# go-distributed/gossip_simulator

Measured on AMD Instinct MI355X. Metric: gossip messages delivered/sec (node) at N=1e9; rounds-to-coverage parity, higher is better.
Workload: dtype u32; 1 GPU; C5-reference-model: single push-flood broadcast per GPU; n=1000000000, fanout=5, fanin=6, delaylow=10, delayhigh=20, ticks=290, status=quiescent, parallelism=trials1

## Files before the change

gossip_simulator_amd/csrc/gs_ctx.cpp:

```cpp
#include "gs_ctx.h"

namespace gs {

namespace {

uint32_t ring_slots(const gs_params& p) { return p.delay_high > 2 ? (uint32_t)p.delay_high : 2u; }

uint32_t ceil_log2(uint64_t x) {
  uint32_t b = 0;
  while ((1ull << b) < x) ++b;
  return b;
}

int check_params(const gs_params* p, bool rumor_trials, std::string& why) {
  if (!p) { why = "params is NULL"; return GS_EINVAL; }
  if (p->n == 0) { why = "n must be >= 1 (simulator.go:240 panics on rand.Intn(0))"; return GS_EINVAL; }
  if (p->n > 0x7FFFFFFFull) { why = "n must be < 2^31"; return GS_EINVAL; }
  if (p->delay_high <= p->delay_low) {
    why = "delayhigh must exceed delaylow (simulator.go:167 panics on rand.Intn(<=0))";
    return GS_EINVAL;
  }
  if (p->fanout < 0 || p->fanin < 0 || p->fanout > 255 || p->fanin > 255) {
    why = "fanout/fanin must be in [0, 255]";
    return GS_EINVAL;
  }
  if (ring_slots(*p) > 4096) { why = "delayhigh must be <= 4096"; return GS_EINVAL; }
  if (p->model > GS_MODEL_RUMOR) {
    why = "model must be GS_MODEL_FLOOD, GS_MODEL_PUSHPULL or GS_MODEL_RUMOR";
    return GS_EINVAL;
  }
  if (p->model == GS_MODEL_RUMOR && (p->rumor_k < 1 || p->rumor_k > 255)) {
    why = "GS_MODEL_RUMOR needs 1 <= rumor_k <= 255, not " + std::to_string(p->rumor_k);
    return GS_EINVAL;
  }
  if (p->model == GS_MODEL_RUMOR && (p->rumor_mode & ~(GS_RUMOR_BLIND | GS_RUMOR_COIN | GS_RUMOR_PULL))) {
    why = "GS_MODEL_RUMOR: rumor_mode " + std::to_string(p->rumor_mode) +
          " has a bit that is none of GS_RUMOR_BLIND, GS_RUMOR_COIN, GS_RUMOR_PULL";
    return GS_EINVAL;
  }
  if (p->model == GS_MODEL_RUMOR && p->trials > 1 && !rumor_trials) {
    why = "GS_MODEL_RUMOR with trials > 1: the rumor model runs one trial per context (gs_create_trials makes a batch)";
    return GS_EINVAL;
  }
  if (p->trials > 1 && ((uint64_t)p->trials << std::max<uint32_t>(kFineLog, ceil_log2(p->n))) > 0x7FFFFFFFull) {
    why = "trials x 2^ceil(log2 n) must be < 2^31 (batch fewer trials per context)";
    return GS_EINVAL;
  }
  return GS_OK;
}

bool alloc_trial_rows(gs_ctx* c, size_t tb, size_t cb) {
  return dev_malloc((void**)&c->bt.d_tstat, tb) == hipSuccess &&
         hipHostMalloc((void**)&c->bt.h_tstat, tb) == hipSuccess && grow(c->bt.chk, cb);
}

void release_trials(gs_ctx* c) {
  if (c->bt.d_tstat) (void)dev_free(c->bt.d_tstat);
  if (c->bt.h_tstat) (void)hipHostFree(c->bt.h_tstat);
  release(c->bt.chk);
}

int alloc_window(gs_ctx* c) {
  const DevState& s = c->st;
  WinState& w = c->ws;
  w.n = s.n;
  w.W = s.W;
  w.nfine = (uint32_t)((s.n + kFineNodes - 1) >> kFineLog);
  w.ncoarse = (w.nfine + 255) / 256;
  w.R = s.R;
  w.delay_low = s.delay_low;
  w.delay_span = s.delay_span;
  w.kd = s.kd;
  w.kc = s.kc;
  w.key = s.key;
  w.base = (uint32_t)c->lo;
  w.tlog = c->tlog;
  w.tmask = c->tlog >= 32 ? ~0u : (1u << c->tlog) - 1;
  w.tnodes = c->trials > 1 && c->tlog <= kCoarseShift && !c->shard ? (uint32_t)c->p.n : 0u;
  w.G = c->G;
  w.rank = c->rank;
  w.seg_per = (uint32_t)c->seg_per;
  w.csub = kCoarseSub;
  w.noxcd = getenv("GS_PART2_NOXCD") ? 1u : 0u;
  {
    const char* xp = getenv("GS_XPAIR");
    w.nopair = xp && atoi(xp) == 0 ? 1u : 0u;
  }
  w.ccap_end = nullptr;
  w.csrc = nullptr;
  if (c->shard) {
    w.owner = 1;
    w.obins = 256 / c->G;
    w.oseg_q = (uint32_t)(c->seg_per >> kFineLog);
    w.oseg_magic = 0xFFFFFFFFu / w.oseg_q;
    if (dev_malloc(&c->wn.d_rtab, kRtabWords * 8) != hipSuccess ||
        hipHostMalloc((void**)&c->wn.h_rtab, kRtabWords * 8) != hipSuccess)
      return fail(c, GS_ENOMEM, "cannot allocate the shard's receive layout");
  }
  auto al = [](size_t b) { return (b + 255) & ~(size_t)255; };
  const size_t units = (size_t)kMaxWindow * w.nfine + 1;
  const size_t b_fc = al((size_t)w.R * w.nfine * 4), b_units = al(units * 8),
               b_small = al(kRegions * 8) * 2 + al((kRegions + 1) * 8) + al((kRegions + 1) * 4) + al(kMaxWindow * 8),
               b_fhist = al(((size_t)w.ncoarse * 256 + 1) * 8), b_fbase = al(((size_t)w.nfine + 1) * 8),
               b_ffill = al((size_t)w.nfine * 8),
               b_sst = al((size_t)kStatShards * kMaxWindow * kStatFields * 8),
               b_rlcnt = al((size_t)w.nfine * 4),
               b_tsum = al((size_t)w.ncoarse * kMaxWindow * 8) + al(((size_t)w.ncoarse + 1) * 8);
  const size_t total = b_fc + 2 * b_units + b_small + b_fhist + b_fbase + b_ffill + b_sst + b_rlcnt + b_tsum;
  if (dev_malloc(&c->wn.d_win, total) != hipSuccess)
    return fail(c, GS_ENOMEM, "cannot allocate window-engine buffers");
  const size_t flist = (size_t)w.R * w.nfine * kFineNodes * 2;
  if (dev_malloc(&c->wn.d_flist, flist) != hipSuccess)
    return fail(c, GS_ENOMEM, "cannot allocate " + std::to_string(flist >> 20) + " MiB of fire lists");
  char* q = (char*)c->wn.d_win;
  w.fcount = (uint32_t*)q; q += b_fc;
  w.usize = (unsigned long long*)q; q += b_units;
  w.unit_off = (unsigned long long*)q; q += b_units;
  w.chist = (unsigned long long*)q; q += al(kRegions * 8);
  w.cfill = (unsigned long long*)q; q += al(kRegions * 8);
  w.ccap = (unsigned long long*)q; q += al((kRegions + 1) * 8);
  w.tprefix = (uint32_t*)q; q += al((kRegions + 1) * 4);
  w.tfires = (unsigned long long*)q;
  q = (char*)c->wn.d_win + b_fc + 2 * b_units + b_small;
  w.fhist = (unsigned long long*)q; q += b_fhist;
  w.fstart = (unsigned long long*)q; q += b_fbase;
  w.ffill = (unsigned long long*)q; q += b_ffill;
  w.sstats = (unsigned long long*)q; q += b_sst;
  w.rlcnt = (uint32_t*)q; q += b_rlcnt;
  w.tsum = (unsigned long long*)q; q += al((size_t)w.ncoarse * kMaxWindow * 8);
  w.toff = (unsigned long long*)q; q += al(((size_t)w.ncoarse + 1) * 8);
  if (dev_malloc(&c->wn.d_rlmsg, (size_t)w.nfine * kRolledCap * 4) != hipSuccess)
    return fail(c, GS_ENOMEM, "cannot allocate the rolled-receipt lists");
  w.rlmsg = (uint32_t*)c->wn.d_rlmsg;
  w.dbg = nullptr;
  if (getenv("GS_STAMPS") && dev_malloc(&w.dbg, kDbgWords * 8) == hipSuccess)
    (void)hipMemset(w.dbg, 0, kDbgWords * 8);
  w.flist = (uint16_t*)c->wn.d_flist;
  c->wn.fcount_bytes = (size_t)w.R * w.nfine * 4;
  if (hipMemsetAsync(c->wn.d_win, 0, total, c->stream) != hipSuccess)
    return fail(c, GS_EDEVICE, "memset of window buffers failed");
  c->wn.misc_words = std::max<size_t>(4096, (size_t)c->G * kMaxWindow + 64);
  if (hipHostMalloc((void**)&c->wn.h_cap, (kRegions + 1) * 8) != hipSuccess ||
      hipHostMalloc((void**)&c->wn.h_misc, c->wn.misc_words * 8) != hipSuccess ||
      hipHostMalloc((void**)&c->wn.h_err, 64) != hipSuccess)
    return fail(c, GS_ENOMEM, "cannot allocate pinned window buffers");
  if (c->trials > 1) {
    if (!alloc_trial_rows(c, (size_t)c->trials * kMaxWindow * kTStatFields * 4, 0))
      return fail(c, GS_ENOMEM, "cannot allocate per-trial counters");
    w.tstat = c->bt.d_tstat;
  }
  return GS_OK;
}

void release_window(gs_ctx* c) {
  WinEngine& e = c->wn;
  for (void* p : {e.d_win, e.d_flist, e.d_rlmsg, (void*)e.d_rtab, (void*)c->ws.dbg})
    if (p) (void)dev_free(p);
  for (Buf* b : {&e.gmap, &e.cmsg, &e.fmsg, &e.tmp}) release(*b);
  for (void* p : {(void*)e.h_cap, (void*)e.h_misc, (void*)e.h_err, (void*)e.h_rtab})
    if (p) (void)hipHostFree(p);
}

int ctx_setup(gs_ctx* c, const gs_params* params, int device, bool shard, uint32_t G, uint32_t rank,
              std::string& why) {
  c->p = *params;
  c->p.device = device;
  c->dev = device;
  int ndev = 0;
  if (hipGetDeviceCount(&ndev) != hipSuccess || ndev <= 0) {
    why = "no HIP device visible (libgossip_hip needs an MI355X)";
    return GS_EDEVICE;
  }
  if (c->dev < 0 || c->dev >= ndev) {
    why = "device " + std::to_string(c->dev) + " out of range (" + std::to_string(ndev) + " visible)";
    return GS_EDEVICE;
  }
  hipDeviceProp_t prop;
  if (hipSetDevice(c->dev) != hipSuccess || hipGetDeviceProperties(&prop, c->dev) != hipSuccess ||
      strncmp(prop.gcnArchName, "gfx950", 6) != 0) {
    why = "device " + std::to_string(c->dev) + " is not gfx950";
    return GS_EDEVICE;
  }
  if (hipStreamCreateWithFlags(&c->own, hipStreamNonBlocking) != hipSuccess) {
    why = "cannot create a stream";
    return GS_EDEVICE;
  }
  c->stream = c->own;
  DevState& s = c->st;
  const uint32_t stride0 = (uint32_t)std::max(c->p.fanout, c->p.fanin);
  c->pp = c->p.model == GS_MODEL_PUSHPULL;
  c->rumor = c->p.model == GS_MODEL_RUMOR;
  c->pp_l2_only = (c->p.flags & GS_FLAG_PP_L2_ONLY) != 0;
  c->trials = std::max<uint32_t>(1, c->p.trials);
  c->ntot = c->p.n;
  if (c->trials > 1) {
    c->tlog = std::max<uint32_t>(kFineLog, ceil_log2(c->p.n));
    c->ntot = (uint64_t)c->trials << c->tlog;
  }
  c->shard = shard;
  c->G = G;
  c->rank = rank;
  if (shard && c->rumor) {
    why = "GS_MODEL_RUMOR runs on one device: no node-range shards";
    return GS_EINVAL;
  }
  if (shard) {
    if (c->pp && !pp_rslot_packed(stride0)) {
      why = "push-pull node-range shards need rows of at most 16 slots (bottom-up rounds)";
      return GS_EINVAL;
    }
    c->seg_per = (((c->p.n + G - 1) / G) + kFineNodes - 1) & ~(uint64_t)(kFineNodes - 1);
// ... 486 lines not shown
```

gossip_simulator_amd/csrc/gs_internal.h:

```cpp
#pragma once
#include <stdint.h>
#include <hip/hip_runtime.h>

#include <algorithm>
#include <vector>

#include "gs_devmem.h"
#include "gs_rng.h"

namespace gs {

inline uint32_t grid_for(uint64_t items, uint32_t per_block, uint32_t cap) {
  return (uint32_t)std::min<uint64_t>((items + per_block - 1) / per_block, cap);
}

constexpr uint32_t kWave = 64;
constexpr uint32_t kChunkNodesLog = 12;
constexpr uint32_t kChunkWords = 64;
constexpr uint32_t kShards = 32;
constexpr uint32_t kCounterStride = 16;
constexpr uint32_t kStatFields = 8;
constexpr uint32_t kStatSlots = 4096;
constexpr uint32_t kListCap = 1024;
constexpr uint32_t kTickBlock = 256;
constexpr uint32_t kTickGridMax = 2048;

enum Stat : uint32_t {
  ST_FIRED = 0, ST_SENT = 1, ST_MSGS = 2, ST_RECV = 3, ST_CRASH = 4, ST_SCHED = 5,
  ST_ERR = 6, ST_RSVD = 7
};

enum Mode : int {
  MODE_FLOOD = 0,
  MODE_COUNT = 1,
  MODE_RESOLVE = 2
};

struct DevState {
  const uint8_t* deg;
  const uint32_t* ids;
  unsigned long long* recv;
  unsigned long long* crash;
  uint32_t* rollw;
  uint32_t* cnt;
  unsigned long long* ring;
  uint32_t* cflag;
  uint32_t* clist;
  uint32_t* ccount;
  unsigned long long* stats;
  uint32_t* err;
  unsigned long long* grecv;
  unsigned long long* gcrash;
  uint64_t gbase;
  uint64_t n, W;
  uint32_t C, CS, R, stride;
  uint32_t stride_magic;
  int32_t delay_low;
  uint32_t delay_span;
  int32_t kd, kc;
  int32_t check_crashed;
  int32_t sharded;
  uint32_t lo, hi;
  uint32_t chunk_lo, chunk_hi;
  Key key;
};

constexpr uint32_t kFineLog = 14;
constexpr uint32_t kFineNodes = 1u << kFineLog;
constexpr uint32_t kCoarseShift = kFineLog + 8;
constexpr uint32_t kMaxWindow = 16;
constexpr uint32_t kCoarseSub = 8;
constexpr uint32_t kRegions = 256 * kCoarseSub;
constexpr uint32_t kWinMaxRing = 256;
constexpr uint32_t kWinMaxStride = 32;
constexpr uint32_t kEmptyMsg = 0xFFFFFFFFu;
constexpr uint32_t kSrcShift = 56;
constexpr unsigned long long kSrcMask = (1ull << kSrcShift) - 1;
#ifndef GS_PART_TILE
#define GS_PART_TILE 16384
#endif
constexpr uint32_t kPartTile = GS_PART_TILE;
constexpr uint32_t kRolledCap = 1024;
constexpr uint32_t kBitTicks = 10;
constexpr uint32_t kXRoundNodes = 2048;
constexpr uint32_t kWinSlotsPerBucket = 1u << 16;

struct WinCtl {
  uint32_t t, L, tnext, tend;
  uint32_t poll, pbase, stop, lmax;
  unsigned long long Tn, T;
  unsigned long long recv, crashed, pending, cover, max_ticks;
  unsigned long long cmsg_cap, fmsg_cap;
  unsigned long long xs_cap, xr_cap;
};
constexpr uint32_t kStageWords = 8 + 16 * 8;

struct WinState {
  const uint8_t* deg;
  const uint32_t* ids;
  unsigned long long* recv;
  unsigned long long* crash;
  uint32_t* rollw;
  uint32_t* rlmsg;
  uint32_t* rlcnt;
  unsigned long long* stats;
  uint32_t* err;
  uint32_t* fcount;
  uint16_t* flist;
  unsigned long long* usize;
  unsigned long long* unit_off;
  unsigned long long* tfires;
  uint32_t* gmap;
  const uint32_t* pk;
  uint32_t noxcd;
  uint32_t nopair;
  uint32_t* cmsg;
  uint32_t* fmsg;
  unsigned long long* chist;
  unsigned long long* ccap;
  const unsigned long long* ccap_end;
  unsigned long long* cfill;
  uint32_t* tprefix;
  unsigned long long* fhist;
  unsigned long long* fstart;
  unsigned long long* ffill;
  unsigned long long* tsum;
  unsigned long long* toff;
  unsigned long long* sstats;
  unsigned long long* dbg;
  uint32_t* tstat;
  uint32_t tofs;
  WinCtl* ctl;
  unsigned long long* stage;
  uint32_t lstride;
  uint32_t slots;
  uint32_t csub;
  const uint32_t* const* csrc;
  uint32_t owner;
  uint32_t obins;
  uint32_t oseg_q, oseg_magic;
  uint32_t abort_on_err;
  uint32_t G, rank;
  uint32_t seg_per;
  uint32_t dd;
  uint32_t guard;
  uint32_t solo;
  unsigned long long* gcnt;
  unsigned long long* glay;
  unsigned long long* wstat;
  uint64_t nglob;
  uint64_t n, W;
  uint32_t nfine, ncoarse, R, stride, stride_magic;
  int32_t delay_low;
  uint32_t delay_span;
  int32_t kd, kc;
  uint32_t base;
  uint32_t tlog, tmask;
  uint32_t tnodes;
  Key key;
};
constexpr uint32_t kStatShards = 32;
constexpr uint32_t kStampPhases = 10;
constexpr uint32_t kXStamp0 = 2 * kStampPhases;
constexpr uint32_t kDbgWords = kXStamp0 + 8;
enum TStat : uint32_t { TS_FIRED = 0, TS_SENT = 1, TS_DEAD = 2, TS_RECV = 3, TS_CRASH = 4, TS_HOT = 5 };
constexpr uint32_t kTStatFields = 8;

__host__ __device__ __forceinline__ void node_key(uint32_t tlog, uint32_t tmask, const Key& key,
                                                  uint64_t g, uint32_t kind, uint32_t& node,
                                                  uint32_t& c3) {
  node = (uint32_t)(g & tmask);
  c3 = ctr3(kind, key.trial + (uint32_t)(g >> tlog));
}

constexpr uint32_t kErrArrivals = 4;
constexpr uint32_t kErrCoarse = 8;
constexpr uint32_t kErrFine = 16;
constexpr uint32_t kErrAbort = 32;
constexpr uint32_t kErrNoMem = 64;
constexpr uint32_t kDDRow = kRegions + 4;
constexpr uint32_t kDDWStat = kMaxWindow * kStatFields + 8;
constexpr size_t kRtabWords = 4 * (kRegions + 1) + 260;
constexpr size_t kRtabTotal = kRtabWords - 1;

hipError_t win_units(const WinState& w, uint32_t t0, uint32_t L, hipStream_t s);
hipError_t win_cut(const WinState& w, unsigned long long budget, hipStream_t s);
hipError_t win_unitscan(const WinState& w, hipStream_t s);
// ... 230 lines not shown
```

gossip_simulator_amd/csrc/gs_win_resolve.hip:

```cpp
#include <algorithm>

#include "gs_win_dev.h"

namespace gs {
namespace {

constexpr uint32_t kResolveMaxBuckets = 256;
constexpr uint32_t kSmallMax = 256;
#ifndef GS_SMALL_BLOCK
#define GS_SMALL_BLOCK 512
#endif
constexpr uint32_t kSmallBlock = GS_SMALL_BLOCK;
#ifndef GS_ROLLED_BLOCK
#define GS_ROLLED_BLOCK 256
#endif
constexpr uint32_t kRolledBlock = GS_ROLLED_BLOCK;

constexpr uint32_t kBitWords = kFineNodes / 32;
struct ResolveLds {
  union {
    struct {
      uint32_t b1[kBitTicks][kBitWords];
      uint2 cr0[kBitWords];
    };
    struct {
      uint32_t cnt[kFineNodes];
      uint32_t recv[kBitWords];
      uint32_t crash[kBitWords];
      uint32_t nrecv[kBitWords];
      uint32_t ncrash[kBitWords];
    };
  };
  uint32_t fc[kWinMaxRing];
  uint32_t st[kMaxWindow][4];
  uint32_t dead[kMaxWindow];
  uint32_t blist[kResolveMaxBuckets];
  unsigned long long bstart[kResolveMaxBuckets];
  uint32_t bcnt[kResolveMaxBuckets];
  uint32_t ndup;
  uint32_t ninf;
  uint32_t err;
  uint32_t nb;
  uint32_t cls;
  unsigned long long stamp[2][kStampPhases];
  unsigned long long tlast;
};
static_assert(kBitTicks <= kMaxWindow, "window ticks fit the message format");
static_assert(sizeof(uint32_t) * kFineNodes <= sizeof(((ResolveLds*)0)->cnt), "the infection list fits");

__device__ __forceinline__ void stamp(const WinState& w, ResolveLds& sm, uint32_t i) {
  if (w.dbg && threadIdx.x == 0) {
    const unsigned long long t = __builtin_amdgcn_s_memtime();
    if (i) sm.stamp[sm.cls][i] += t - sm.tlast;
    sm.tlast = t;
  }
}

#if defined(GS_RESOLVE_PROBE) && GS_RESOLVE_PROBE == 1
#define GS_RESOLVE_CR0(loc) make_uint2(0u, 0u)
#else
#define GS_RESOLVE_CR0(loc) sm.cr0[(loc) >> 5]
#endif


__device__ __forceinline__ void resolve_node(const WinState& w, ResolveLds& sm, uint32_t f,
                                             uint32_t loc, uint32_t kk, uint32_t ones, uint32_t t,
                                             uint32_t& cm, uint32_t& cr, uint32_t& cc, uint32_t& cs) {
  const uint32_t bit = 1u << (loc & 31), wi = loc >> 5;
  if (sm.crash[wi] & bit) return;
  const uint64_t g = (uint64_t)w.base + (f << kFineLog) + loc;
  uint32_t u, c3order;
  node_key(w.tlog, w.tmask, w.key, g, K_ORDER, u, c3order);
  const uint32_t pos = ones ? first_crash(u, t, kk, ones, c3order, w.key.k0, w.key.k1) : kk + 1;
  cm += pos <= kk ? pos : kk;
  if (pos > 1 && !(sm.recv[wi] & bit)) {
    atomicOr(&sm.recv[wi], bit);
    ++cr;
    uint32_t c3delay;
    node_key(w.tlog, w.tmask, w.key, g, K_DELAY, u, c3delay);
    const uint32_t off = fire_offset(w.delay_low, w.delay_span,
                                     philox(u, t, 0, c3delay, w.key.k0, w.key.k1).x);
    const uint32_t s = (t + off) % w.R;
    const uint32_t at = atomicAdd(&sm.fc[s], 1u);
    w.flist[((size_t)s * w.nfine + f) * kFineNodes + at] = (uint16_t)loc;
    ++cs;
  }
  if (pos <= kk) {
    atomicOr(&sm.crash[wi], bit);
    ++cc;
  }
}

template <class Src>
__device__ __forceinline__ void resolve_tick(const WinState& w, ResolveLds& sm, uint32_t f,
                                             const Src& src, uint32_t lo, uint32_t hi, uint32_t k,
                                             uint32_t t) {
  const uint32_t tid = threadIdx.x;
  for (uint32_t p = lo + tid; p < hi; p += kResolveBlock) {
    const uint32_t m = src[p];
    if (msg_tick(m) != k) continue;
    const uint32_t old = atomicAdd(&sm.cnt[msg_loc(m)], 1u + (((m >> kRoll0Fine) & 1u) << 16));
    if ((old & 0xFFFFu) == 0xFFFFu) sm.err = 1;
  }
  __syncthreads();
  uint32_t arr = 0, cm = 0, cr = 0, cc = 0, cs = 0;
  for (uint32_t p = lo + tid; p < hi; p += kResolveBlock) {
    const uint32_t m = src[p];
    if (msg_tick(m) != k) continue;
    const uint32_t loc = msg_loc(m);
    const uint32_t kk = atomicExch(&sm.cnt[loc], 0u);
    arr += kk & 0xFFFFu;
    if (kk) resolve_node(w, sm, f, loc, kk & 0xFFFFu, kk >> 16, t, cm, cr, cc, cs);
  }
  if (arr != cm) atomicAdd(&sm.st[k][0], arr - cm);
  if (cr) atomicAdd(&sm.st[k][1], cr);
  if (cc) atomicAdd(&sm.st[k][2], cc);
  (void)cs;
  __syncthreads();
}

__device__ __forceinline__ void flush_counts(const WinState& w, ResolveLds& sm, uint32_t (&acc_ni)[kBitTicks / 2],
                                             uint32_t L, uint32_t trial) {
#pragma unroll
  for (uint32_t k = 0; k < kBitTicks; ++k) {
    if (k >= L) continue;
    const uint32_t sr = wave_sum((acc_ni[k / 2] >> (16 * (k & 1))) & 0xFFFFu);
    if (lane_id() == 0 && sr) atomicAdd(&sm.st[k][1], sr);
  }
#pragma unroll
  for (uint32_t k = 0; k < kBitTicks / 2; ++k) acc_ni[k] = 0;
  __syncthreads();
  const uint32_t tid = threadIdx.x;
  if (tid < L * 3) {
    const uint32_t k = tid / 3, fld = tid - k * 3;
    const uint32_t v = sm.st[k][fld];
    unsigned long long* row = shard_row(w, k);
    if (v && fld == 0) atomicAdd(&row[ST_MSGS], 0ull - (unsigned long long)v);
    if (v && fld == 1) {
      atomicAdd(&row[ST_RECV], (unsigned long long)v);
      atomicAdd(&row[ST_SCHED], (unsigned long long)v);
    }
    if (v && fld == 2) atomicAdd(&row[ST_CRASH], (unsigned long long)v);
    if (v && trial != ~0u) atomicAdd(&w.tstat[((size_t)trial * kMaxWindow + w.tofs + k) * kTStatFields + TS_DEAD + fld], v);
    sm.st[k][fld] = 0;
  }
  __syncthreads();
}

__device__ __forceinline__ void resolve_body(const WinState& w, uint32_t t0, uint32_t L) {
  __shared__ ResolveLds sm;
  const uint32_t tid = threadIdx.x, G = gridDim.x;
  L = win_live(w, t0, L);
  if (!L) return;
  static_assert(kBitWords == kResolveBlock, "one bit word per thread");
  static_assert(kWinMaxRing <= kResolveBlock, "one ring slot per thread");
  if (tid < kMaxWindow * 4) (&sm.st[0][0])[tid] = 0;
  if (tid == 0) { sm.nb = 0; sm.cls = 0; }
  if (tid < 2 * kStampPhases) (&sm.stamp[0][0])[tid] = 0;
  __syncthreads();
  {
    const uint32_t f = blockIdx.x + tid * G;
    const unsigned long long fl = tid < kResolveMaxBuckets && f < w.nfine ? w.ffill[f] : 0ull;
    const bool ne = fl > kSmallMax;
    const uint32_t at = wave_append(&sm.nb, ne);
    if (ne) {
      sm.blist[at] = f;
      sm.bstart[at] = w.fstart[f];
      sm.bcnt[at] = (uint32_t)fl;
    }
  }
  __syncthreads();
  const uint32_t nb = sm.nb;
  stamp(w, sm, 0);
  uint32_t fB = 0, MB = 0;
  unsigned long long mbB = 0;
  auto next_bucket = [&](uint32_t j) { fB = sm.blist[j]; mbB = sm.bstart[j]; MB = sm.bcnt[j]; };
  if (nb > 0) next_bucket(0);
  uint32_t* rwg = (uint32_t*)w.recv;
  uint32_t* cwg = (uint32_t*)w.crash;
  uint32_t acc_ni[kBitTicks / 2];
#pragma unroll
  for (uint32_t k = 0; k < kBitTicks / 2; ++k) acc_ni[k] = 0;
  static_assert(kBitTicks % 2 == 0 && 32 * kResolveMaxBuckets < 65536, "two 16-bit counts per register");
  constexpr uint32_t kU = 8;
  constexpr uint32_t kBatch = kResolveBlock * kU;
  auto ld = [&](const uint32_t* gm, uint32_t M, uint32_t p0, uint32_t (&m)[kU]) {
#pragma unroll
    for (uint32_t u = 0; u < kU; ++u) {
      const uint32_t p = p0 + u * kResolveBlock + tid;
      m[u] = *reinterpret_cast<const uint32_t*>(reinterpret_cast<const char*>(gm) + ((p < M ? p : M - 1) << 2));
    }
  };
  uint32_t pm[kU], p_recv0 = 0, p_crash0 = 0, p_roll0 = 0, p_fcv = 0;
  bool p_in = false;
  auto prefetch = [&](uint32_t f, uint32_t M, unsigned long long mb) {
    const uint64_t wi = ((uint64_t)(f << kFineLog) >> 5) + tid;
    const bool in = wi < w.W * 2;
    const uint64_t wc = in ? wi : w.W * 2 - 1;
    p_in = in;
    p_recv0 = rwg[wc];
    p_crash0 = cwg[wc];
    p_roll0 = w.rollw[wc];
    p_fcv = w.fcount[(size_t)(tid < w.R ? tid : 0u) * w.nfine + f];
    ld(w.fmsg + mb, M, 0, pm);
// ... 94 lines not shown
    if (i + 1 < nb) prefetch(fB, MB, mbB);
    if (tid == 0) w.rlcnt[f] = sm.err == 3 ? 0u : min(sm.ndup, kRolledCap);
    stamp(w, sm, 3);
    uint32_t rw = recv0, cw = crash0;
    if (sm.err != 3) {
      if (tid < L && sm.dead[tid]) atomicAdd(&sm.st[tid][0], sm.dead[tid]);
      uint32_t infk[kBitTicks], ninf = 0;
      const uint32_t plain = ~(crash0 | rollw);
#pragma unroll
      for (uint32_t k = 0; k < kBitTicks; ++k) {
        infk[k] = 0;
        if (k >= L) continue;
        const uint32_t infS = sm.b1[k][tid] & plain & ~rw;
        rw |= infS;
        infk[k] = infS;
      }
      stamp(w, sm, 4);
#pragma unroll
      for (uint32_t k = 0; k < kBitTicks; ++k) {
        const uint32_t ni = __popc(infk[k]);
        acc_ni[k / 2] += ni << (16 * (k & 1));
        ninf += ni;
      }
      stamp(w, sm, 5);
      __syncthreads();
      stamp(w, sm, 6);
      auto bcast = [&](uint32_t x) {
        const uint32_t loc = msg_loc(x), t = t0 + msg_tick(x);
        const uint32_t off = fire_offset(w.delay_low, w.delay_span,
                                         philox(knode0 + loc, t, 0, c3delay, w.key.k0, w.key.k1).x);
        const uint32_t slot = (t + off) % w.R;
        const uint32_t pos = atomicAdd(&sm.fc[slot], 1u);
        w.flist[((size_t)slot * w.nfine + f) * kFineNodes + pos] = (uint16_t)loc;
      };
      uint32_t* inf = &sm.cnt[0];
      {
        uint32_t pre = 0, tot = 0;
#pragma unroll
        for (uint32_t b = 0; b < 9; ++b) {
          const unsigned long long bal = __ballot((ninf >> b) & 1u);
          pre += lanes_below(bal) << b;
          tot += (uint32_t)__popcll(bal) << b;
        }
        uint32_t base = 0;
        if (tot && lane_id() == 0) base = atomicAdd(&sm.ninf, tot);
        uint32_t at = __builtin_amdgcn_readfirstlane(base) + pre;
#pragma unroll
        for (uint32_t k = 0; k < kBitTicks; ++k)
          for (uint32_t x = k < L ? infk[k] : 0u; x; x &= x - 1)
            inf[at++] = (tid * 32 + __builtin_ctz(x)) | (k << kFineLog);
      }
      __syncthreads();
      stamp(w, sm, 7);
      const uint32_t ni_all = sm.ninf;
      for (uint32_t q = tid; q < ni_all; q += kResolveBlock) bcast(inf[q]);
    } else {
      __syncthreads();
      uint4* c4 = reinterpret_cast<uint4*>(sm.cnt);
      for (uint32_t q = tid; q < kFineNodes / 4; q += kResolveBlock) c4[q] = make_uint4(0, 0, 0, 0);
      sm.recv[tid] = recv0;
      sm.crash[tid] = crash0;
      sm.nrecv[tid] = 0;
      sm.ncrash[tid] = 0;
      __syncthreads();
      for (uint32_t k = 0; k < L; ++k) resolve_tick(w, sm, f, gm, 0, M, k, t0 + k);
      rw = sm.recv[tid] | sm.nrecv[tid];
      cw = sm.crash[tid] | sm.ncrash[tid];
      if (tid == 0 && sm.err == 1) atomicOr(w.err, kErrArrivals);
    }
    __syncthreads();
    stamp(w, sm, 8);
    if (in) {
      if (rw != recv0) rwg[wi] = rw;
      if (cw != crash0) cwg[wi] = cw;
    }
    if (tid < w.R) w.fcount[(size_t)tid * w.nfine + f] = sm.fc[tid];
    stamp(w, sm, 9);
    if (w.dbg && tid == 0) sm.stamp[sm.cls][0] += 1;
    if (w.tstat) flush_counts(w, sm, acc_ni, L, (uint32_t)(((uint64_t)w.base + node0) >> w.tlog));
  }
  if (w.dbg && tid < 2 * kStampPhases) atomicAdd(&w.dbg[tid], (&sm.stamp[0][0])[tid]);
  if (!w.tstat) flush_counts(w, sm, acc_ni, L, ~0u);
}
__global__ __launch_bounds__(kResolveBlock, GS_RESOLVE_WAVES) void k_resolve(const WinState w, uint32_t t0, uint32_t L) {
  resolve_body(w, t0, L);
}
__global__ __launch_bounds__(kResolveBlock, GS_RESOLVE_WAVES) void k_resolve_m(const WinState* __restrict__ ws,
                                                                                uint32_t L) {
  resolve_body(ws[blockIdx.y], 0u, L);
}

template <uint32_t E, bool ROLLED>
__device__ __forceinline__ void resolve_small_bucket(const WinState& w, uint32_t t0, uint32_t L, uint32_t f,
                                                     const uint32_t* gm, unsigned long long M,
                                                     uint32_t (*st)[kMaxWindow][4], uint32_t* skw,
                                                     uint32_t* fcw) {
  constexpr uint32_t N = 64 * E;
  const uint32_t lane = threadIdx.x & 63, wv = threadIdx.x >> 6;
  {
    const bool consume = !ROLLED && w.ctl;
    const uint32_t s0 = t0 % w.R;
    for (uint32_t s = lane; s < w.R; s += 64)
      fcw[s] = consume && (s + w.R - s0) % w.R < L ? 0u : w.fcount[(size_t)s * w.nfine + f];
    uint32_t knode0, c3order;
    node_key(w.tlog, w.tmask, w.key, (uint64_t)w.base + (f << kFineLog), K_ORDER, knode0, c3order);
    const uint32_t c3delay = (c3order & 0xFFFFFFu) | (K_DELAY << 24);
    uint32_t key[E];
#pragma unroll
    for (uint32_t r = 0; r < E; ++r) {
      const uint32_t i = lane * E + r;
      key[r] = ~0u;
      if (i < M) {
        const uint32_t m = gm[i];
        key[r] = (msg_loc(m) << 5) | (msg_tick(m) << 1) | ((m >> kRoll0Fine) & 1u);
        if (!ROLLED && ((m >> kRoll0Fine) & 1u)) w.rollw[((f << kFineLog) + msg_loc(m)) >> 5] = 0u;
      }
    }
#pragma unroll
    for (uint32_t k = 2; k <= N; k <<= 1)
#pragma unroll
      for (uint32_t j = k >> 1; j > 0; j >>= 1) {
        if (j >= E) {
#pragma unroll
          for (uint32_t r = 0; r < E; ++r) {
            const uint32_t i = lane * E + r;
            const uint32_t o = __shfl_xor(key[r], j / E, 64);
            const bool keep_min = ((i & j) == 0) == ((i & k) == 0);
            key[r] = keep_min ? min(key[r], o) : max(key[r], o);
          }
        } else {
#pragma unroll
          for (uint32_t r = 0; r < E; ++r) {
            if (r & j) continue;
            const bool up = ((lane * E + r) & k) == 0;
            const uint32_t a = key[r], b = key[r | j];
            key[r] = up ? min(a, b) : max(a, b);
            key[r | j] = up ? max(a, b) : min(a, b);
          }
        }
      }
#pragma unroll
    for (uint32_t r = 0; r < E; ++r) skw[lane * E + r] = key[r];
    wave_lds_sync();
    uint32_t* rwg = (uint32_t*)w.recv;
    uint32_t* cwg = (uint32_t*)w.crash;
    bool any_inf = false;
    uint32_t head = 0;
#pragma unroll
    for (uint32_t r = 0; r < E; ++r) {
      const uint32_t i = lane * E + r;
      if (key[r] != ~0u && !(i > 0 && (skw[i - 1] >> 5) == (key[r] >> 5))) head |= 1u << r;
    }
#pragma unroll 1
    for (uint32_t r = 0; r < E; ++r) {
      if (!((head >> r) & 1u)) continue;
      const uint32_t i = lane * E + r;
      const uint32_t loc = skw[i] >> 5;
      const uint32_t wi = ((f << kFineLog) + loc) >> 5, bit = 1u << (loc & 31), u = knode0 + loc;
      const uint32_t cw = cwg[wi];
      bool rv = (rwg[wi] & bit) != 0, cr = (cw & bit) != 0, inf = false;
      uint32_t tinf = 0;
      for (uint32_t q = i; q < N;) {
        const uint32_t e = skw[q];
        if ((e >> 5) != loc) break;
        const uint32_t k = (e >> 1) & (kMaxWindow - 1), t = t0 + k;
        uint32_t c = 0, ones = 0;
        for (; q < N && (skw[q] >> 1) == (e >> 1); ++q) {
          ++c;
          ones += skw[q] & 1u;
        }
        if (cr) {
          atomicAdd(&st[wv][k][0], c);
// ... 22 lines not shown
        w.flist[((size_t)slot * w.nfine + f) * kFineNodes + pos] = (uint16_t)loc;
      }
    }
    wave_lds_sync();
    if (__ballot(any_inf)) {
      for (uint32_t s = lane; s < w.R; s += 64) w.fcount[(size_t)s * w.nfine + f] = fcw[s];
    } else if (consume && lane < L) {
      w.fcount[(size_t)((t0 + lane) % w.R) * w.nfine + f] = 0;
    }
    if (w.tstat) {
      wave_lds_sync();
      if (lane < L * 3) {
        const uint32_t k = lane / 3, fld = lane - k * 3;
        const uint32_t v = st[wv][k][fld];
        const uint32_t trial = (uint32_t)(((uint64_t)w.base + (f << kFineLog)) >> w.tlog);
        if (v) atomicAdd(&w.tstat[((size_t)trial * kMaxWindow + w.tofs + k) * kTStatFields + TS_DEAD + fld], v);
      }
    }
  }
}

template <bool ROLLED>
__device__ __forceinline__ void resolve_small_body(const WinState& w, uint32_t t0, uint32_t L) {
  constexpr uint32_t kWaves = (ROLLED ? kRolledBlock : kSmallBlock) / 64;
  constexpr uint32_t kEmax = ROLLED ? 16 : 4;
  __shared__ uint32_t st[kWaves][kMaxWindow][4];
  __shared__ uint32_t sk[kWaves][64 * kEmax];
  __shared__ uint32_t fcw[kWaves][kWinMaxRing];
  const uint32_t tid = threadIdx.x, wv = tid >> 6;
  static_assert(kWaves * kMaxWindow * 4 == kWaves * 64, "one counter per thread");
  static_assert(kRolledCap == 64 * 16, "the rolled bodies cover 1..kRolledCap");
  const uint32_t f = __builtin_amdgcn_readfirstlane(blockIdx.x * kWaves + wv);
  unsigned long long M = 0;
  const uint32_t* gm = nullptr;
  if (f < w.nfine) {
    if (ROLLED) {
      M = w.rlcnt[f];
      gm = w.rlmsg + (size_t)f * kRolledCap;
    } else {
      M = w.ffill[f];
      gm = w.fmsg + w.fstart[f];
    }
  }
  L = win_live(w, t0, L);
  if (!L) return;
  (&st[0][0][0])[tid] = 0;
  __syncthreads();
  if (M > 0 && M <= 64) resolve_small_bucket<1, ROLLED>(w, t0, L, f, gm, M, st, sk[wv], fcw[wv]);
  else if (M > 64 && M <= 256) resolve_small_bucket<4, ROLLED>(w, t0, L, f, gm, M, st, sk[wv], fcw[wv]);
  else if (ROLLED && M > 256 && M <= 512)
    resolve_small_bucket<ROLLED ? 8 : 1, ROLLED>(w, t0, L, f, gm, M, st, sk[wv], fcw[wv]);
  else if (ROLLED && M > 512 && M <= kRolledCap)
    resolve_small_bucket<ROLLED ? 16 : 1, ROLLED>(w, t0, L, f, gm, M, st, sk[wv], fcw[wv]);
  if (ROLLED && M && (threadIdx.x & 63) == 0) w.rlcnt[f] = 0;
  if (!ROLLED && w.ctl && !(M > 0 && M <= 256) && f < w.nfine && (threadIdx.x & 63) < L)
    w.fcount[(size_t)((t0 + (threadIdx.x & 63)) % w.R) * w.nfine + f] = 0;
  __syncthreads();
  if (tid < L * 3) {
    const uint32_t k = tid / 3, fld = tid - k * 3;
    uint32_t v = 0;
    for (uint32_t q = 0; q < kWaves; ++q) v += st[q][k][fld];
    unsigned long long* row = shard_row(w, k);
    if (v && fld == 0) atomicAdd(&row[ST_MSGS], 0ull - (unsigned long long)v);
    if (v && fld == 1) {
      atomicAdd(&row[ST_RECV], (unsigned long long)v);
      atomicAdd(&row[ST_SCHED], (unsigned long long)v);
    }
    if (v && fld == 2) atomicAdd(&row[ST_CRASH], (unsigned long long)v);
  }
}
template <bool ROLLED>
__global__ __launch_bounds__(ROLLED ? kRolledBlock : kSmallBlock) void k_resolve_small(const WinState w, uint32_t t0,
                                                                                       uint32_t L) {
  resolve_small_body<ROLLED>(w, t0, L);
}
template <bool ROLLED>
__global__ __launch_bounds__(ROLLED ? kRolledBlock : kSmallBlock) void k_resolve_small_m(
    const WinState* __restrict__ ws, uint32_t L) {
  resolve_small_body<ROLLED>(ws[blockIdx.y], 0u, L);
}

}

hipError_t win_resolve(const WinState& w, uint32_t t0, uint32_t L, hipStream_t s) {
  const uint32_t cus = device_cus();
  static const uint32_t per_cu = [] { const char* e = getenv("GS_RESOLVE_PER_CU"); return e ? (uint32_t)std::max(atoi(e), 1) : 2u; }();
  uint32_t G = std::min<uint32_t>(w.nfine, per_cu * cus);
  G = std::max<uint32_t>(G, (w.nfine + kResolveMaxBuckets - 1) / kResolveMaxBuckets);
  const uint32_t gs = (w.nfine + kSmallBlock / 64 - 1) / (kSmallBlock / 64);
  hipLaunchKernelGGL(k_resolve_small<false>, dim3(gs), dim3(kSmallBlock), 0, s, w, t0, L);
  static_assert(kSmallMax == 64 * 4, "the two bodies cover 1..kSmallMax");
  hipLaunchKernelGGL(k_resolve, dim3(G), dim3(kResolveBlock), 0, s, w, t0, L);
  hipLaunchKernelGGL(k_resolve_small<true>, dim3((w.nfine + kRolledBlock / 64 - 1) / (kRolledBlock / 64)),
                     dim3(kRolledBlock), 0, s, w, t0, L);
  return hipGetLastError();
}

hipError_t win_resolve_g(const WinGroup& g, uint32_t L, hipStream_t s) {
  const uint32_t cus = device_cus();
  uint32_t G = std::min<uint32_t>(g.nfine_max, (2 * cus + g.M - 1) / g.M);
  G = std::max<uint32_t>(G, (g.nfine_max + kResolveMaxBuckets - 1) / kResolveMaxBuckets);
  const uint32_t gs = (g.nfine_max + kSmallBlock / 64 - 1) / (kSmallBlock / 64);
  hipLaunchKernelGGL(k_resolve_small_m<false>, dim3(gs, g.M), dim3(kSmallBlock), 0, s, g.wr, L);
  hipLaunchKernelGGL(k_resolve_m, dim3(G, g.M), dim3(kResolveBlock), 0, s, g.wr, L);
  hipLaunchKernelGGL(k_resolve_small_m<true>, dim3((g.nfine_max + kRolledBlock / 64 - 1) / (kRolledBlock / 64), g.M),
                     dim3(kRolledBlock), 0, s, g.wr, L);
  return hipGetLastError();
}

}
```

Measured before the change: 84.56 billion msgs/s.

## Add slimmer-LDS resolve kernel with overflow fallback to a large-bucket pass

Introduces a new resolve kernel whose shared-memory footprint is trimmed (a smaller infection list unioned with the crash/roll words, dead counts packed into 6-bit fields), so three workgroups fit per CU instead of two. It also prefetches the next bucket's state. Buckets whose duplicate-receipt list overflows are recorded in a new global list and handled by a separate large-bucket kernel running the old per-tick path. This is enabled by default with more blocks per CU. The risks are an extra launch, chunked infection processing when the list exceeds its capacity, and more complex control flow.

```diff
diff --git a/gossip_simulator_amd/csrc/gs_ctx.cpp b/gossip_simulator_amd/csrc/gs_ctx.cpp
--- a/gossip_simulator_amd/csrc/gs_ctx.cpp
+++ b/gossip_simulator_amd/csrc/gs_ctx.cpp
@@ -104,7 +104,7 @@
                b_fhist = al(((size_t)w.ncoarse * 256 + 1) * 8), b_fbase = al(((size_t)w.nfine + 1) * 8),
                b_ffill = al((size_t)w.nfine * 8),
                b_sst = al((size_t)kStatShards * kMaxWindow * kStatFields * 8),
-               b_rlcnt = al((size_t)w.nfine * 4),
+               b_rlcnt = al((size_t)w.nfine * 4) + al(((size_t)w.nfine + 2) * 4),
                b_tsum = al((size_t)w.ncoarse * kMaxWindow * 8) + al(((size_t)w.ncoarse + 1) * 8);
   const size_t total = b_fc + 2 * b_units + b_small + b_fhist + b_fbase + b_ffill + b_sst + b_rlcnt + b_tsum;
   if (dev_malloc(&c->wn.d_win, total) != hipSuccess)
@@ -126,7 +126,8 @@
   w.fstart = (unsigned long long*)q; q += b_fbase;
   w.ffill = (unsigned long long*)q; q += b_ffill;
   w.sstats = (unsigned long long*)q; q += b_sst;
-  w.rlcnt = (uint32_t*)q; q += b_rlcnt;
+  w.rlcnt = (uint32_t*)q; q += al((size_t)w.nfine * 4);
+  w.lgl = (uint32_t*)q; q += al(((size_t)w.nfine + 2) * 4);
   w.tsum = (unsigned long long*)q; q += al((size_t)w.ncoarse * kMaxWindow * 8);
   w.toff = (unsigned long long*)q; q += al(((size_t)w.ncoarse + 1) * 8);
   if (dev_malloc(&c->wn.d_rlmsg, (size_t)w.nfine * kRolledCap * 4) != hipSuccess)
diff --git a/gossip_simulator_amd/csrc/gs_internal.h b/gossip_simulator_amd/csrc/gs_internal.h
--- a/gossip_simulator_amd/csrc/gs_internal.h
+++ b/gossip_simulator_amd/csrc/gs_internal.h
@@ -103,6 +103,7 @@
   uint32_t* rollw;
   uint32_t* rlmsg;
   uint32_t* rlcnt;
+  uint32_t* lgl;
   unsigned long long* stats;
   uint32_t* err;
   uint32_t* fcount;
diff --git a/gossip_simulator_amd/csrc/gs_win_resolve.hip b/gossip_simulator_amd/csrc/gs_win_resolve.hip
--- a/gossip_simulator_amd/csrc/gs_win_resolve.hip
+++ b/gossip_simulator_amd/csrc/gs_win_resolve.hip
@@ -48,7 +48,8 @@
 static_assert(kBitTicks <= kMaxWindow, "window ticks fit the message format");
 static_assert(sizeof(uint32_t) * kFineNodes <= sizeof(((ResolveLds*)0)->cnt), "the infection list fits");
 
-__device__ __forceinline__ void stamp(const WinState& w, ResolveLds& sm, uint32_t i) {
+template <class Lds>
+__device__ __forceinline__ void stamp(const WinState& w, Lds& sm, uint32_t i) {
   if (w.dbg && threadIdx.x == 0) {
     const unsigned long long t = __builtin_amdgcn_s_memtime();
     if (i) sm.stamp[sm.cls][i] += t - sm.tlast;
@@ -119,7 +120,8 @@
   __syncthreads();
 }
 
-__device__ __forceinline__ void flush_counts(const WinState& w, ResolveLds& sm, uint32_t (&acc_ni)[kBitTicks / 2],
+template <class Lds>
+__device__ __forceinline__ void flush_counts(const WinState& w, Lds& sm, uint32_t (&acc_ni)[kBitTicks / 2],
                                              uint32_t L, uint32_t trial) {
 #pragma unroll
   for (uint32_t k = 0; k < kBitTicks; ++k) {
@@ -380,12 +382,299 @@
   if (w.dbg && tid < 2 * kStampPhases) atomicAdd(&w.dbg[tid], (&sm.stamp[0][0])[tid]);
   if (!w.tstat) flush_counts(w, sm, acc_ni, L, ~0u);
 }
-__global__ __launch_bounds__(kResolveBlock, GS_RESOLVE_WAVES) void k_resolve(const WinState w, uint32_t t0, uint32_t L) {
+__global__ __launch_bounds__(kResolveBlock, GS_RESOLVE_WAVES) void k_resolve2(const WinState w, uint32_t t0, uint32_t L) {
   resolve_body(w, t0, L);
 }
-__global__ __launch_bounds__(kResolveBlock, GS_RESOLVE_WAVES) void k_resolve_m(const WinState* __restrict__ ws,
-                                                                                uint32_t L) {
+__global__ __launch_bounds__(kResolveBlock, GS_RESOLVE_WAVES) void k_resolve2_m(const WinState* __restrict__ ws,
+                                                                                 uint32_t L) {
   resolve_body(ws[blockIdx.y], 0u, L);
+}
+
+constexpr uint32_t kInfCap = 6656;
+constexpr uint32_t kResolveWaves3 = 6;
+struct ResolveLds3 {
+  uint32_t b1[kBitTicks][kBitWords];
+  union {
+    uint2 cr0[kBitWords];
+    uint32_t inf[kInfCap];
+  };
+  uint32_t fc[kWinMaxRing];
+  uint32_t st[kMaxWindow][4];
+  uint32_t dead[kMaxWindow];
+  uint32_t blist[kResolveMaxBuckets];
+  unsigned long long bstart[kResolveMaxBuckets];
+  uint32_t bcnt[kResolveMaxBuckets];
+  uint32_t ndup;
+  uint32_t ninf;
+  uint32_t err;
+  uint32_t nb;
+  uint32_t cls;
+  unsigned long long stamp[2][kStampPhases];
+  unsigned long long tlast;
+};
+static_assert(sizeof(ResolveLds3) <= 53 * 1024, "three workgroups per CU");
+static_assert(kBitTicks * 6 <= 64, "6-bit dead counts per tick in one register pair");
+
+__device__ __forceinline__ void resolve3_body(const WinState& w, uint32_t t0, uint32_t L) {
+  __shared__ ResolveLds3 sm;
+  const uint32_t tid = threadIdx.x, G = gridDim.x;
+  L = win_live(w, t0, L);
+  if (!L) return;
+  if (tid < kMaxWindow * 4) (&sm.st[0][0])[tid] = 0;
+  if (tid == 0) { sm.nb = 0; sm.cls = 0; }
+  if (tid < 2 * kStampPhases) (&sm.stamp[0][0])[tid] = 0;
+  __syncthreads();
+  {
+    const uint32_t f = blockIdx.x + tid * G;
+    const unsigned long long fl = tid < kResolveMaxBuckets && f < w.nfine ? w.ffill[f] : 0ull;
+    const bool ne = fl > kSmallMax;
+    const uint32_t at = wave_append(&sm.nb, ne);
+    if (ne) {
+      sm.blist[at] = f;
+      sm.bstart[at] = w.fstart[f];
+      sm.bcnt[at] = (uint32_t)fl;
+    }
+  }
+  __syncthreads();
+  const uint32_t nb = sm.nb;
+  stamp(w, sm, 0);
+  uint32_t* rwg = (uint32_t*)w.recv;
+  uint32_t* cwg = (uint32_t*)w.crash;
+  uint32_t acc_ni[kBitTicks / 2];
+#pragma unroll
+  for (uint32_t k = 0; k < kBitTicks / 2; ++k) acc_ni[k] = 0;
+  constexpr uint32_t kU = 4;
+  constexpr uint32_t kBatch = kResolveBlock * kU;
+  auto ld = [&](const uint32_t* gm, uint32_t M, uint32_t p0, uint32_t (&m)[kU]) {
+#pragma unroll
+    for (uint32_t u = 0; u < kU; ++u) {
+      const uint32_t p = p0 + u * kResolveBlock + tid;
+      m[u] = *reinterpret_cast<const uint32_t*>(reinterpret_cast<const char*>(gm) + ((p < M ? p : M - 1) << 2));
+    }
+  };
+  uint32_t pm[kU], p_recv0 = 0, p_crash0 = 0, p_roll0 = 0, p_fcv = 0;
+  bool p_in = false;
+  auto prefetch = [&](uint32_t j) {
+    const uint32_t f = sm.blist[j];
+    const uint64_t wi = ((uint64_t)(f << kFineLog) >> 5) + tid;
+    const bool in = wi < w.W * 2;
+    const uint64_t wc = in ? wi : w.W * 2 - 1;
+    p_in = in;
+    p_recv0 = rwg[wc];
+    p_crash0 = cwg[wc];
+    p_roll0 = w.rollw[wc];
+    p_fcv = w.fcount[(size_t)(tid < w.R ? tid : 0u) * w.nfine + f];
+    ld(w.fmsg + sm.bstart[j], sm.bcnt[j], 0, pm);
+  };
+  if (nb > 0) prefetch(0);
+  for (uint32_t i = 0; i < nb; ++i) {
+    const uint32_t f = sm.blist[i], M = sm.bcnt[i];
+    const uint32_t* gm = w.fmsg + sm.bstart[i];
+    uint32_t m[kU];
+#pragma unroll
+    for (uint32_t u = 0; u < kU; ++u) m[u] = pm[u];
+    const uint32_t node0 = f << kFineLog;
+    const uint64_t wi = ((uint64_t)node0 >> 5) + tid;
+    const bool in = p_in;
+    const uint32_t recv0 = in ? p_recv0 : 0u, crash0 = in ? p_crash0 : 0u, roll0 = in ? p_roll0 : 0u;
+    if (roll0) w.rollw[wi] = 0u;
+    const uint32_t rollw = roll0 & ~crash0;
+#pragma unroll
+    for (uint32_t k = 0; k < kBitTicks; ++k)
+      if (k < L) sm.b1[k][tid] = 0;
+    sm.cr0[tid] = make_uint2(crash0, rollw);
+    if (tid < w.R) sm.fc[tid] = p_fcv;
+    if (tid < kMaxWindow) sm.dead[tid] = 0;
+    if (tid == 0) { sm.ndup = 0; sm.ninf = 0; sm.err = M >= (1u << 28) ? 3 : 0; sm.cls = M >= 1024 ? 1 : 0; }
+    __syncthreads();
+    stamp(w, sm, 1);
+    unsigned long long dd = 0;
+    auto flush_dead = [&]() {
+      while (dd) {
+        const uint32_t b = (uint32_t)__builtin_ctzll(dd) / 6;
+        atomicAdd(&sm.dead[b], (uint32_t)(dd >> (6 * b)) & 63u);
+        dd &= ~(63ull << (6 * b));
+      }
+    };
+    for (uint32_t p0 = 0, nbat = 0; p0 < (sm.err == 3 ? 0u : M); p0 += kBatch, ++nbat) {
+      uint32_t mn[kU];
+      if (p0 + kBatch < M) ld(gm, M, p0 + kBatch, mn);
+      uint2 sp[kU];
+#pragma unroll
+      for (uint32_t u = 0; u < kU; ++u) {
+        const uint32_t loc = msg_loc(m[u]);
+        atomicOr(&sm.b1[msg_tick(m[u])][loc >> 5], 1u << (loc & 31));
+        sp[u] = GS_RESOLVE_CR0(loc);
+      }
+      uint32_t dm = 0;
+#pragma unroll
+      for (uint32_t u = 0; u < kU; ++u) {
+        const uint32_t sh = msg_loc(m[u]) & 31, k = msg_tick(m[u]);
+        const uint32_t valid = p0 + u * kResolveBlock + tid < M ? 1u : 0u;
+        dd += (unsigned long long)((sp[u].x >> sh) & valid) << (6 * k);
+        dm |= ((sp[u].y >> sh) & valid) << u;
+      }
+      if (nbat % 15 == 14) flush_dead();
+      if (__ballot(dm != 0)) {
+        const uint32_t nd = __popc(dm);
+        uint32_t pre = 0, tot = 0;
+#pragma unroll
+        for (uint32_t bb = 0; bb < 3; ++bb) {
+          const unsigned long long bal = __ballot((nd >> bb) & 1u);
+          pre += lanes_below(bal) << bb;
+          tot += (uint32_t)__popcll(bal) << bb;
+        }
+        uint32_t base = 0;
+        if (lane_id() == 0) base = atomicAdd(&sm.ndup, tot);
+        uint32_t at = __builtin_amdgcn_readfirstlane(base) + pre;
+#pragma unroll
+        for (uint32_t u = 0; u < kU; ++u) if ((dm >> u) & 1u) {
+          if (at < kRolledCap) w.rlmsg[(size_t)f * kRolledCap + at] = m[u] & ((1u << 19) - 1);
+          else sm.err = 3;
+          ++at;
+        }
+      }
+#pragma unroll
+      for (uint32_t u = 0; u < kU; ++u) m[u] = mn[u];
+    }
+    flush_dead();
+    stamp(w, sm, 2);
+    __syncthreads();
+    if (i + 1 < nb) prefetch(i + 1);
+    const bool large = sm.err == 3;
+    if (tid == 0) {
+      w.rlcnt[f] = large ? 0u : sm.ndup;
+      if (large) w.lgl[2 + atomicAdd(&w.lgl[0], 1u)] = f;
+    }
+    stamp(w, sm, 3);
+    if (!large) {
+      if (tid < L && sm.dead[tid]) atomicAdd(&sm.st[tid][0], sm.dead[tid]);
+      const uint32_t plain = ~(crash0 | rollw);
+      uint32_t rw = recv0, ninf = 0;
+#pragma unroll
+      for (uint32_t k = 0; k < kBitTicks; ++k) {
+        if (k >= L) continue;
+        const uint32_t infS = sm.b1[k][tid] & plain & ~rw;
+        rw |= infS;
+        const uint32_t ni = __popc(infS);
+        acc_ni[k / 2] += ni << (16 * (k & 1));
+        ninf += ni;
+      }
+      stamp(w, sm, 4);
+      stamp(w, sm, 5);
+      stamp(w, sm, 6);
+      if (in && rw != recv0) rwg[wi] = rw;
+      uint32_t at0;
+      {
+        uint32_t pre = 0, tot = 0;
+#pragma unroll
+        for (uint32_t b = 0; b < 9; ++b) {
+          const unsigned long long bal = __ballot((ninf >> b) & 1u);
+          pre += lanes_below(bal) << b;
+          tot += (uint32_t)__popcll(bal) << b;
+        }
+        uint32_t base = 0;
+        if (tot && lane_id() == 0) base = atomicAdd(&sm.ninf, tot);
+        at0 = __builtin_amdgcn_readfirstlane(base) + pre;
+      }
+      for (uint32_t r0 = 0;; r0 += kInfCap) {
+        uint32_t at = at0 - r0, r = recv0;
+#pragma unroll
+        for (uint32_t k = 0; k < kBitTicks; ++k) {
+          if (k >= L) continue;
+          uint32_t x = sm.b1[k][tid] & plain & ~r;
+          r |= x;
+          for (; x; x &= x - 1, ++at)
+            if (at < kInfCap) sm.inf[at] = (tid * 32 + __builtin_ctz(x)) | (k << kFineLog);
+        }
+        __syncthreads();
+        stamp(w, sm, 7);
+        const uint32_t left = sm.ninf - r0;
+        for (uint32_t q = tid; q < min(left, kInfCap); q += kResolveBlock) {
+          const uint32_t x = sm.inf[q];
+          const uint32_t loc = msg_loc(x), t = t0 + msg_tick(x);
+          uint32_t knode0, c3order;
+          node_key(w.tlog, w.tmask, w.key, (uint64_t)w.base + node0, K_ORDER, knode0, c3order);
+          const uint32_t c3delay = (c3order & 0xFFFFFFu) | (K_DELAY << 24);
+          const uint32_t off = fire_offset(w.delay_low, w.delay_span,
+                                           philox(knode0 + loc, t, 0, c3delay, w.key.k0, w.key.k1).x);
+          const uint32_t slot = (t + off) % w.R;
+          const uint32_t pos = atomicAdd(&sm.fc[slot], 1u);
+          w.flist[((size_t)slot * w.nfine + f) * kFineNodes + pos] = (uint16_t)loc;
+        }
+        if (left <= kInfCap) break;
+        __syncthreads();
+      }
+    }
+    __syncthreads();
+    stamp(w, sm, 8);
+    if (!large && tid < w.R) w.fcount[(size_t)tid * w.nfine + f] = sm.fc[tid];
+    stamp(w, sm, 9);
+    if (w.dbg && tid == 0) sm.stamp[sm.cls][0] += 1;
+    if (w.tstat) flush_counts(w, sm, acc_ni, L, (uint32_t)(((uint64_t)w.base + node0) >> w.tlog));
+  }
+  if (w.dbg && tid < 2 * kStampPhases) atomicAdd(&w.dbg[tid], (&sm.stamp[0][0])[tid]);
+  if (!w.tstat) flush_counts(w, sm, acc_ni, L, ~0u);
+}
+__global__ __launch_bounds__(kResolveBlock, kResolveWaves3) void k_resolve(const WinState w, uint32_t t0, uint32_t L) {
+  resolve3_body(w, t0, L);
+}
+__global__ __launch_bounds__(kResolveBlock, kResolveWaves3) void k_resolve_m(const WinState* __restrict__ ws,
+                                                                             uint32_t L) {
+  resolve3_body(ws[blockIdx.y], 0u, L);
+}
+
+__device__ __forceinline__ void resolve_large_body(const WinState& w, uint32_t t0, uint32_t L) {
+  __shared__ ResolveLds sm;
+  const uint32_t n = w.lgl[0];
+  if (!n) return;
+  const uint32_t tid = threadIdx.x;
+  L = win_live(w, t0, L);
+  if (L) {
+    if (tid < kMaxWindow * 4) (&sm.st[0][0])[tid] = 0;
+    uint32_t acc_ni[kBitTicks / 2];
+#pragma unroll
+    for (uint32_t k = 0; k < kBitTicks / 2; ++k) acc_ni[k] = 0;
+    uint32_t* rwg = (uint32_t*)w.recv;
+    uint32_t* cwg = (uint32_t*)w.crash;
+    for (uint32_t j = blockIdx.x; j < n; j += gridDim.x) {
+      const uint32_t f = w.lgl[2 + j], M = (uint32_t)w.ffill[f];
+      const uint32_t* gm = w.fmsg + w.fstart[f];
+      const uint32_t node0 = f << kFineLog;
+      const uint64_t wi = ((uint64_t)node0 >> 5) + tid;
+      const bool in = wi < w.W * 2;
+      const uint32_t recv0 = in ? rwg[wi] : 0u, crash0 = in ? cwg[wi] : 0u;
+      uint4* c4 = reinterpret_cast<uint4*>(sm.cnt);
+      for (uint32_t q = tid; q < kFineNodes / 4; q += kResolveBlock) c4[q] = make_uint4(0, 0, 0, 0);
+      sm.recv[tid] = recv0;
+      sm.crash[tid] = crash0;
+      if (tid < w.R) sm.fc[tid] = w.fcount[(size_t)tid * w.nfine + f];
+      if (tid == 0) sm.err = 0;
+      __syncthreads();
+      for (uint32_t k = 0; k < L; ++k) resolve_tick(w, sm, f, gm, 0, M, k, t0 + k);
+      const uint32_t rw = sm.recv[tid], cw = sm.crash[tid];
+      if (in) {
+        if (rw != recv0) rwg[wi] = rw;
+        if (cw != crash0) cwg[wi] = cw;
+      }
+      if (tid < w.R) w.fcount[(size_t)tid * w.nfine + f] = sm.fc[tid];
+      if (tid == 0 && sm.err == 1) atomicOr(w.err, kErrArrivals);
+      if (w.tstat) flush_counts(w, sm, acc_ni, L, (uint32_t)(((uint64_t)w.base + node0) >> w.tlog));
+      else __syncthreads();
+    }
+    if (!w.tstat) flush_counts(w, sm, acc_ni, L, ~0u);
+  }
+  __syncthreads();
+  if (tid == 0 && atomicAdd(&w.lgl[1], 1u) == gridDim.x - 1) {
+    w.lgl[0] = 0;
+    w.lgl[1] = 0;
+  }
+}
+__global__ __launch_bounds__(kResolveBlock) void k_resolve_large(const WinState w, uint32_t t0, uint32_t L) {
+  resolve_large_body(w, t0, L);
+}
+__global__ __launch_bounds__(kResolveBlock) void k_resolve_large_m(const WinState* __restrict__ ws, uint32_t L) {
+  resolve_large_body(ws[blockIdx.y], 0u, L);
 }
 
 template <uint32_t E, bool ROLLED>
@@ -574,15 +863,27 @@
 
 }
 
+static bool resolve_occ3() {
+  static const bool on = [] { const char* e = getenv("GS_RESOLVE_OCC3"); return !e || atoi(e) != 0; }();
+  return on;
+}
+
 hipError_t win_resolve(const WinState& w, uint32_t t0, uint32_t L, hipStream_t s) {
   const uint32_t cus = device_cus();
-  static const uint32_t per_cu = [] { const char* e = getenv("GS_RESOLVE_PER_CU"); return e ? (uint32_t)std::max(atoi(e), 1) : 2u; }();
+  const bool occ3 = resolve_occ3();
+  static const uint32_t per_cu_env = [] { const char* e = getenv("GS_RESOLVE_PER_CU"); return e ? (uint32_t)std::max(atoi(e), 1) : 0u; }();
+  const uint32_t per_cu = per_cu_env ? per_cu_env : occ3 ? 6u : 2u;
   uint32_t G = std::min<uint32_t>(w.nfine, per_cu * cus);
   G = std::max<uint32_t>(G, (w.nfine + kResolveMaxBuckets - 1) / kResolveMaxBuckets);
   const uint32_t gs = (w.nfine + kSmallBlock / 64 - 1) / (kSmallBlock / 64);
   hipLaunchKernelGGL(k_resolve_small<false>, dim3(gs), dim3(kSmallBlock), 0, s, w, t0, L);
   static_assert(kSmallMax == 64 * 4, "the two bodies cover 1..kSmallMax");
-  hipLaunchKernelGGL(k_resolve, dim3(G), dim3(kResolveBlock), 0, s, w, t0, L);
+  if (occ3) {
+    hipLaunchKernelGGL(k_resolve, dim3(G), dim3(kResolveBlock), 0, s, w, t0, L);
+    hipLaunchKernelGGL(k_resolve_large, dim3(std::min<uint32_t>(w.nfine, cus)), dim3(kResolveBlock), 0, s, w, t0, L);
+  } else {
+    hipLaunchKernelGGL(k_resolve2, dim3(G), dim3(kResolveBlock), 0, s, w, t0, L);
+  }
   hipLaunchKernelGGL(k_resolve_small<true>, dim3((w.nfine + kRolledBlock / 64 - 1) / (kRolledBlock / 64)),
                      dim3(kRolledBlock), 0, s, w, t0, L);
   return hipGetLastError();
@@ -590,11 +891,18 @@
 
 hipError_t win_resolve_g(const WinGroup& g, uint32_t L, hipStream_t s) {
   const uint32_t cus = device_cus();
-  uint32_t G = std::min<uint32_t>(g.nfine_max, (2 * cus + g.M - 1) / g.M);
+  const bool occ3 = resolve_occ3();
+  uint32_t G = std::min<uint32_t>(g.nfine_max, ((occ3 ? 3 : 2) * cus + g.M - 1) / g.M);
   G = std::max<uint32_t>(G, (g.nfine_max + kResolveMaxBuckets - 1) / kResolveMaxBuckets);
   const uint32_t gs = (g.nfine_max + kSmallBlock / 64 - 1) / (kSmallBlock / 64);
   hipLaunchKernelGGL(k_resolve_small_m<false>, dim3(gs, g.M), dim3(kSmallBlock), 0, s, g.wr, L);
-  hipLaunchKernelGGL(k_resolve_m, dim3(G, g.M), dim3(kResolveBlock), 0, s, g.wr, L);
+  if (occ3) {
+    hipLaunchKernelGGL(k_resolve_m, dim3(G, g.M), dim3(kResolveBlock), 0, s, g.wr, L);
+    hipLaunchKernelGGL(k_resolve_large_m, dim3(std::min<uint32_t>(g.nfine_max, (cus + g.M - 1) / g.M), g.M),
+                       dim3(kResolveBlock), 0, s, g.wr, L);
+  } else {
+    hipLaunchKernelGGL(k_resolve2_m, dim3(G, g.M), dim3(kResolveBlock), 0, s, g.wr, L);
+  }
   hipLaunchKernelGGL(k_resolve_small_m<true>, dim3((g.nfine_max + kRolledBlock / 64 - 1) / (kRolledBlock / 64), g.M),
                      dim3(kRolledBlock), 0, s, g.wr, L);
   return hipGetLastError();
```

New measurement: 86.70 billion msgs/s, median of 6. 1.03x the previous value.
